# vibhatha/cylon

Hardware: AMD Instinct MI355X
Metric: rows/sec distributed inner-join, 1B×1B int64 keys, at 1/2/4/8 MI355X (higher is better)
Workload: dtype int64 keys / float64 payload; 1 GPU; model=distributed inner join (hash), int64 key + 3 float64 cols, global_batch=1000000000, seq_len=4, parallelism=dp1 (local join), rows_per_relation=1000000000, output_rows=1010151446, key_range=990000000

## Files before the change

cylon_amd/csrc/cylon/kernels/radix_join.hip:

```cpp
#include "radix_common.hpp"

namespace cylon {
namespace hip {

struct PartDigit {
  const int64_t *keys;
  int bits;
  int shift;
  uint32_t mask;
  CYLON_DIGIT_COMMON
  __device__ __forceinline__ uint32_t of_key(int64_t k) const { return (part_of(k, bits) >> shift) & mask; }
  __device__ __forceinline__ uint32_t operator()(int64_t i) const { return of_key(keys[i]); }
  __device__ __forceinline__ uint32_t next_of(uint64_t stored, int nshift, uint32_t nmask, uint64_t) const {
    return (part_of((int64_t)stored, bits) >> nshift) & nmask;
  }
};


struct PartDigitN {
  static constexpr bool kNarrow = true;
  const void *keys;
  int kin4;
  const int64_t *base_src;
  unsigned int *bad;
// ... 168 lines not shown
  const int64_t r0 = t * kRPTile;
#pragma unroll
  for (int u = 0; u < kHTItems; ++u) {
    const int64_t i = r0 + u * kHTThreads + threadIdx.x;
    d[u] = t < ntiles && i < n ? digit(i) : 0xffffffffu;
  }
}
template <class Digit>
__global__ __launch_bounds__(kHTThreads) void k_rp_hist_tiles(Digit digit0, int64_t n, uint32_t nb, int64_t ntiles,
                                                              uint16_t *__restrict__ th) {
  Digit digit = digit0;
  digit.init();
  __shared__ unsigned int hist[kRPMaxBuckets];
  uint32_t d[kHTItems];
  ht_load(digit, n, blockIdx.x, ntiles, d);
  for (int64_t t = blockIdx.x; t < ntiles; t += gridDim.x) {
    for (uint32_t p = threadIdx.x; p < nb; p += blockDim.x) hist[p] = 0;
    __syncthreads();
#pragma unroll
    for (int u = 0; u < kHTItems; ++u)
      if (d[u] != 0xffffffffu) atomicAdd(&hist[d[u]], 1u);
    ht_load(digit, n, t + gridDim.x, ntiles, d);
    __syncthreads();
    for (uint32_t p = threadIdx.x; p < nb; p += blockDim.x) th[t * nb + p] = (uint16_t)hist[p];
    __syncthreads();
  }
}

constexpr int64_t kTsChunk = 512;

__global__ void k_ts_chunk_sums(const uint16_t *__restrict__ th, uint32_t nb, int64_t ntiles,
                                uint32_t *__restrict__ csum) {
  const int64_t c = blockIdx.x, t0 = c * kTsChunk, t1 = t0 + kTsChunk < ntiles ? t0 + kTsChunk : ntiles;
  const uint32_t p = threadIdx.x;
  if (p >= nb) return;
  uint32_t acc = 0;
#pragma unroll 8
  for (int64_t t = t0; t < t1; ++t) acc += th[t * nb + p];
  csum[c * nb + p] = acc;
}

__global__ __launch_bounds__(kRPThreads) void k_ts_chunk_prefix(const uint32_t *__restrict__ csum, uint32_t nb,
                                                                int64_t nchunks, uint32_t *__restrict__ cpre,
                                                                uint32_t *__restrict__ bbase) {
  __shared__ uint32_t wsum[kRPWaves];
  constexpr int B = 16;
  const uint32_t p = threadIdx.x;
  uint32_t acc = 0;
  if (p < nb)
    for (int64_t c0 = 0; c0 < nchunks; c0 += B) {
      uint32_t x[B];
#pragma unroll
      for (int u = 0; u < B; ++u) x[u] = c0 + u < nchunks ? csum[(c0 + u) * nb + p] : 0u;
#pragma unroll
      for (int u = 0; u < B; ++u)
        if (c0 + u < nchunks) {
          cpre[(c0 + u) * nb + p] = acc;
          acc += x[u];
        }
    }
  const uint32_t base = rp_block_exscan<kRPWaves>(p < nb ? acc : 0u, wsum);
  if (p < nb) bbase[p] = base;
}

__global__ void k_ts_offsets(const uint16_t *__restrict__ th, const uint32_t *__restrict__ cpre,
                             const uint32_t *__restrict__ bbase, uint32_t nb, int64_t ntiles,
                             uint32_t *__restrict__ off, const uint32_t *__restrict__ extra) {
  const int64_t c = blockIdx.x, t0 = c * kTsChunk, t1 = t0 + kTsChunk < ntiles ? t0 + kTsChunk : ntiles;
  const uint32_t p = threadIdx.x;
  if (p >= nb) return;
  uint32_t acc = cpre[c * nb + p] + bbase[p] + (extra != nullptr ? extra[p] : 0u);
#pragma unroll 8
  for (int64_t t = t0; t < t1; ++t) {
    off[t * nb + p] = acc;
    acc += th[t * nb + p];
  }
}



template <class Digit, bool W8, int THREADS, int RANK, bool XT = false, bool SLOT = false>
__global__ __launch_bounds__(THREADS) __attribute__((amdgpu_waves_per_eu(4))) void k_rows_pass(
    Digit digit0, int nbits, uint32_t nbuckets, ColSet cols, int64_t n, int64_t rows_per_block, int64_t nblocks,
    const int64_t *__restrict__ bh_scan, TileSched lb) {
  constexpr int WAVES = THREADS / kWave;
  constexpr int TILE = THREADS * kRPItems;
  constexpr int BPT = (kRPMaxBuckets + THREADS - 1) / THREADS;
  Digit digit = digit0;
  digit.init();
  bool narrow_bad = false;
  static_assert(WAVES * kRPMaxBuckets * 2 + TILE * 4 <= TILE * 8, "ranking scratch must fit the stage");
  constexpr bool TICKET = XT || SLOT;
  static_assert(!(XT && SLOT), "one tile schedule");
  static_assert(!SLOT || RANK == kRankBlockAtomic, "slot mode ranks with block atomics (counts in bcnt)");
  const int xhome = TICKET ? xcc_id() : 0;
  __shared__ int64_t running[kRPMaxBuckets];
  __shared__ uint32_t toff[kRPMaxBuckets + 1];
  __shared__ uint64_t ustage[TILE];
  __shared__ uint32_t wsum[WAVES];
  uint16_t *wcnt = reinterpret_cast<uint16_t *>(ustage);
  constexpr bool STABLE = RANK != kRankBlockAtomic;
  uint32_t *bcnt = reinterpret_cast<uint32_t *>(ustage);
  static_assert(WAVES * kRPMaxBuckets * 2 >= kRPMaxBuckets * 4, "block counters must fit the wave counters");
  uint32_t *sdig = reinterpret_cast<uint32_t *>(wcnt + WAVES * kRPMaxBuckets);
  uint8_t *st = reinterpret_cast<uint8_t *>(ustage);
  __shared__ int64_t s_next;
  __shared__ int64_t s_tend[2], s_tr0[2];
  __shared__ int s_tb[2];
  int par = 0;
  bool order_bad = false;
  __shared__ uint32_t tp[SLOT ? kSlotMaxSeg : 1], sss[SLOT ? kSlotMaxSeg : 1], sse[SLOT ? kSlotMaxSeg : 1];
  __shared__ int64_t s_tix, s_thi;
  auto sl_take = [&](int slot) {
    const int64_t t = s_tix;
    if (t >= s_thi) {
      s_tr0[slot] = INT64_MAX / 4;
      s_tend[slot] = 0;
      s_tb[slot] = 0;
      return;
    }
    s_tix = t + ((int64_t)gridDim.x - (blockIdx.x & (kXcds - 1)) + kXcds - 1) / kXcds;
    const int g = sl_segment(tp, lb.sl_nseg, t);
    const int64_t gend = (int64_t)sse[g];
    const int64_t r0 = (int64_t)sss[g] + (t - (int64_t)tp[g]) * TILE;
    s_tr0[slot] = r0;
    s_tend[slot] = r0 + TILE < gend ? r0 + TILE : gend;
    s_tb[slot] = (g >> lb.sl_gshift) * (int)nbuckets * lb.sl_B + (g & lb.sl_gmask);
  };

  const int64_t b = blockIdx.x;
  int64_t begin, end;
  if (SLOT) {
    for (int i = threadIdx.x; i < lb.sl_nseg; i += THREADS) {
      tp[i] = lb.sl_tpre[i];
      sss[i] = lb.sl_ss[i];
      sse[i] = lb.sl_se[i];
    }
    if (threadIdx.x == 0) {
      const int x = blockIdx.x & (kXcds - 1);
      const int g0 = lb.sl_nseg * x / kXcds, g1 = lb.sl_nseg * (x + 1) / kXcds;
      s_tix = (int64_t)lb.sl_tpre[g0] + blockIdx.x / kXcds;
      s_thi = lb.sl_tpre[g1];
    }
    __syncthreads();
    if (threadIdx.x == 0) {
      sl_take(0);
      sl_take(1);
    }
    __syncthreads();
    begin = s_tr0[0];
    end = INT64_MAX / 4;
  } else if (TICKET) {
    if (threadIdx.x == 0) s_next = xt_claim(lb, xhome, TILE, n);
    __syncthreads();
    begin = s_next;
    end = n;
  } else {
    for (uint32_t p = threadIdx.x; p < nbuckets; p += blockDim.x) running[p] = bh_scan[(int64_t)p * nblocks + b];
    begin = b * rows_per_block;
    end = (begin + rows_per_block < n) ? begin + rows_per_block : n;
  }
  const int wave = threadIdx.x / kWave;
  const int lane = lane_id();
  const uint64_t lt = lanemask_lt();
  uint16_t *mycnt = wcnt + wave * nbuckets;
  const int wrow = wave * kWave * kRPItems;

  using KVT = typename std::conditional<Digit::kNarrow, uint32_t, uint64_t>::type;
  KVT kv[kRPItems];
  auto load_key = [&](int64_t i) -> KVT {
    const uint64_t raw = digit.key_at(i);
    if constexpr (Digit::kNarrow) {
      narrow_bad |= digit.too_wide(raw);
      return (KVT)digit.narrow(raw);
    } else {
      return (KVT)raw;
    }
  };
#pragma unroll
  for (int k = 0; k < kRPItems; ++k) {
    const int64_t i = begin + wrow + k * kWave + lane;
    if (i < (SLOT ? s_tend[0] : end)) kv[k] = load_key(i);
  }
  for (int64_t tile = begin, next = 0; tile < end; tile = next) {
    next = tile + TILE;
    const int cnt = SLOT ? (int)(s_tend[par] - tile) : (int)((end - tile) < TILE ? (end - tile) : TILE);
    const uint32_t xoff = XT && threadIdx.x < nbuckets ? lb.xt_off[(tile / TILE) * nbuckets + threadIdx.x] : 0u;
    uint32_t pl[kRPItems];
#pragma unroll
    for (int k = 0; k < kRPItems; ++k) {
      const bool act = wrow + k * kWave + lane < cnt;
      if constexpr (Digit::kNarrow) pl[k] = act ? digit.of_offset(kv[k]) : 0xffffffffu;
      else pl[k] = act ? digit.of_key((int64_t)kv[k]) : 0xffffffffu;
    }
    if (STABLE) {
      for (uint32_t q = threadIdx.x; q < WAVES * nbuckets; q += blockDim.x) wcnt[q] = 0;
    } else {
      for (uint32_t q = threadIdx.x; q < nbuckets; q += blockDim.x) bcnt[q] = 0;
    }
    __syncthreads();
    if (!STABLE) {
#pragma unroll
      for (int k = 0; k < kRPItems; ++k)
        if (pl[k] != 0xffffffffu) pl[k] |= atomicAdd(&bcnt[pl[k]], 1u) << 16;
    } else if (RANK == kRankWaveAtomic) {
      uint32_t *myw = reinterpret_cast<uint32_t *>(mycnt);
#pragma unroll
      for (int k = 0; k < kRPItems; ++k)
        if (pl[k] != 0xffffffffu) {
          const uint32_t p = pl[k], sh = (p & 1u) * 16u;
          pl[k] |= ((atomicAdd(&myw[p >> 1], 1u << sh) >> sh) & 0xffffu) << 16;
        }
    } else
#pragma unroll
    for (int k = 0; k < kRPItems; ++k) {
      const bool active = pl[k] != 0xffffffffu;
      const uint32_t p = active ? pl[k] : 0u;
      uint64_t m = __ballot(active);
      for (int bit = 0; bit < nbits; ++bit) {
        const uint32_t x = (p >> bit) & 1u;
        const uint64_t bb = __ballot(x);
        m &= x ? bb : ~bb;
      }
      const uint32_t rank = (uint32_t)__popcll(m & lt);
      uint32_t base = 0;
      if (active) base = mycnt[p];
      __builtin_amdgcn_wave_barrier();
      if (active && (m & lt) == 0) mycnt[p] = (uint16_t)(base + (uint32_t)__popcll(m));
      __builtin_amdgcn_wave_barrier();
      pl[k] = active ? (((base + rank) << 16) | p) : 0xffffffffu;
    }
    __syncthreads();
    uint32_t sl_c = 0, sl_base = 0;
    if (SLOT && threadIdx.x < nbuckets) {
      sl_c = STABLE ? 0u : bcnt[threadIdx.x];
      if (sl_c) sl_base = atomicAdd(&lb.sl_cursor[(int64_t)s_tb[par] + (int64_t)threadIdx.x * lb.sl_B], sl_c);
    }
    {
      uint32_t loc[BPT];
      uint32_t total = 0;
#pragma unroll
      for (int i = 0; i < BPT; ++i) {
        const uint32_t p = threadIdx.x * BPT + i;
        loc[i] = total;
        uint32_t run = 0;
        if (p < nbuckets) {
          if (STABLE) {
#pragma unroll
            for (int w = 0; w < WAVES; ++w) {
              const uint32_t c = wcnt[w * nbuckets + p];
              wcnt[w * nbuckets + p] = (uint16_t)run;
              run += c;
            }
          } else {
            run = bcnt[p];
          }
        }
        total += run;
      }
      const uint32_t ex = rp_block_exscan<WAVES>(total, wsum);
#pragma unroll
      for (int i = 0; i < BPT; ++i) {
        const uint32_t p = threadIdx.x * BPT + i;
        if (p < nbuckets) toff[p] = ex + loc[i];
      }
      if (threadIdx.x == THREADS - 1) toff[nbuckets] = ex + total;
    }
    __syncthreads();
#pragma unroll
    for (int k = 0; k < kRPItems; ++k) {
      if (pl[k] == 0xffffffffu) continue;
      const uint32_t p = pl[k] & 0xffffu;
      const uint32_t pos = toff[p] + (STABLE ? (uint32_t)wcnt[wave * nbuckets + p] : 0u) + (pl[k] >> 16);
      sdig[pos] = (p << 16) | (uint32_t)(wrow + k * kWave + lane);
      pl[k] = pos;
    }
    if (XT && threadIdx.x < nbuckets) running[threadIdx.x] = xoff;
    if (SLOT && threadIdx.x < nbuckets) {
      const bool fits = (int64_t)sl_base + sl_c <= lb.sl_slot;
      if (sl_c && !fits) atomicOr(lb.sl_overflow, 1u);
      running[threadIdx.x] = fits ? ((int64_t)s_tb[par] + (int64_t)threadIdx.x * lb.sl_B) * lb.sl_slot + sl_base
                                  : lb.sl_nslots * lb.sl_slot;
    }
    __syncthreads();
    constexpr bool PACKDST = false;
    using DstT = typename std::conditional<SLOT, uint32_t, int64_t>::type;
    DstT dst[kRPItems];
#define RP_DEST(q) \
  ((SLOT && PACKDST) ? running[(uint32_t)dst[q] >> 16] + (int64_t)((uint32_t)dst[q] & 0xffffu) : (int64_t)dst[q])
#pragma unroll
    for (int q = 0; q < kRPItems; ++q) {
      const int j = threadIdx.x + q * THREADS;
      if (j < cnt) {
        const uint32_t e = sdig[j], p = e >> 16;
        if constexpr (SLOT && PACKDST) dst[q] = (p << 16) | (uint32_t)(j - (int)toff[p]);
        else dst[q] = (DstT)(running[p] + (j - (int64_t)toff[p]));
        if (cols.check_order && j > 0) {
          const uint32_t f = sdig[j - 1];
          order_bad |= (f >> 16) == p && f > e;
        }
      }
    }
    __syncthreads();
    uint64_t v[kRPItems];
#pragma unroll
    for (int k = 0; k < kRPItems; ++k) v[k] = kv[k];
#pragma unroll 1
    for (int c = 0; c < cols.n; ++c) {
      const int w = cols.width[c];
      uint8_t *out = cols.out[c];
      const uint64_t x = c == 0 ? cols.key_xor : 0ull;
      if (TICKET && c + 1 == cols.n && threadIdx.x == 0) {
        if (!SLOT) s_next = xt_claim(lb, xhome, TILE, n);
      }
      const bool n4 = Digit::kNarrow && c == 0;
      if (n4) {
#pragma unroll
        for (int k = 0; k < kRPItems; ++k)
          if (pl[k] != 0xffffffffu) stw<false>(st, pl[k], 4, v[k] & 0xffffffffull);
      } else {
#pragma unroll
        for (int k = 0; k < kRPItems; ++k)
          if (pl[k] != 0xffffffffu) stw<W8>(st, pl[k], w, v[k] ^ x);
      }
      __syncthreads();
      if (TICKET && c + 1 == cols.n) next = SLOT ? s_tr0[par ^ 1] : s_next;
      if (c + 1 < cols.n) {
        const uint8_t *in = cols.in[c + 1];
        const int w1 = cols.width[c + 1];
        if (in == nullptr) {
#pragma unroll
          for (int k = 0; k < kRPItems; ++k) v[k] = (uint64_t)(tile + wrow + k * kWave + lane);
        } else {
#pragma unroll
          for (int k = 0; k < kRPItems; ++k)
            if (pl[k] != 0xffffffffu) v[k] = ldw<W8>(in, tile + wrow + k * kWave + lane, w1);
        }
      } else {
#pragma unroll
        for (int k = 0; k < kRPItems; ++k) {
          const int64_t i = next + wrow + k * kWave + lane;
          if (i < (SLOT ? s_tend[par ^ 1] : end)) kv[k] = load_key(i);
        }
      }
      if (kNdDigit<Digit> && c == 0 && cols.nd_out != nullptr) {
#pragma unroll
        for (int q = 0; q < kRPItems; ++q) {
          const int j = threadIdx.x + q * THREADS;
          if (j < cnt) {
            const uint64_t kv0 = ldw<W8>(st, j, w);
            const int64_t o = RP_DEST(q);
            stw<W8>(out, o, w, kv0);
            if constexpr (kNdDigit<Digit>)
              cols.nd_out[o] = (uint16_t)digit.next_of(kv0, cols.nd_shift, cols.nd_mask, cols.nd_sub);
          }
        }
      } else if (n4) {
#pragma unroll
        for (int q = 0; q < kRPItems; ++q) {
          const int j = threadIdx.x + q * THREADS;
          if (j < cnt) stw<false>(out, RP_DEST(q), 4, ldw<false>(st, j, 4));
        }
      } else {
#pragma unroll
        for (int q = 0; q < kRPItems; ++q) {
          const int j = threadIdx.x + q * THREADS;
          if (j < cnt) stw<W8>(out, RP_DEST(q), w, ldw<W8>(st, j, w));
        }
      }
      __syncthreads();
    }
#undef RP_DEST
    if (!TICKET)
      for (uint32_t p = threadIdx.x; p < nbuckets; p += blockDim.x) running[p] += toff[p + 1] - toff[p];
    if (SLOT) {
      par ^= 1;
      if (threadIdx.x == 0) sl_take(par ^ 1);
    }
  }
  if (order_bad) atomicOr(cols.order_bad, 1);
  if (Digit::kNarrow && narrow_bad) digit.report_bad();
}

template <class Digit, bool W8, int RANK, bool XT = false, int LBM = 0>
__global__ __launch_bounds__(kRPThreads) __attribute__((amdgpu_waves_per_eu(8))) void k_rows_pass_lean(
    Digit digit, int nbits, uint32_t nbuckets, ColSet cols, int64_t n, int64_t rows_per_block, int64_t nblocks,
    const int64_t *__restrict__ bh_scan, TileSched lb) {
  constexpr int THREADS = kRPThreads, WAVES = THREADS / kWave, TILE = THREADS * kRPItems;
  constexpr bool LBIN = (LBM & 2) != 0, CNT = (LBM & 1) != 0;
  static_assert(LBM == 0 || (XT && (std::is_same<Digit, ImageDigit>::value || std::is_same<Digit, PartDigit>::value)),
                "look-back passes are XT sort / hash-partition passes");
  constexpr int MAXB = LBM ? kLbMaxBuckets : kRPMaxBuckets;
  constexpr int BPT = (MAXB + THREADS - 1) / THREADS;
  static_assert(WAVES * MAXB * 2 + TILE * 4 <= TILE * 8, "ranking scratch must fit the stage");
  __shared__ int64_t running[MAXB];
  __shared__ uint32_t toff[MAXB + 1];
  __shared__ uint64_t ustage[TILE];
  __shared__ uint32_t wsum[WAVES];
  __shared__ uint32_t s_C[LBIN ? kLbChunks + 1 : 1], s_TP[LBIN ? kLbChunks + 2 : 1];
  __shared__ uint32_t lcnt[CNT ? kLbChunks * kLbMaxBuckets / 2 : 1];
  constexpr bool STABLE = RANK != kRankBlockAtomic;
  uint16_t *wcnt = reinterpret_cast<uint16_t *>(ustage);
  uint32_t *bcnt = reinterpret_cast<uint32_t *>(ustage);
  uint32_t *sdig = reinterpret_cast<uint32_t *>(wcnt + WAVES * MAXB);
  uint8_t *st = reinterpret_cast<uint8_t *>(ustage);
  __shared__ int64_t s_next;
  bool order_bad = false;
  (void)nbits;
  constexpr bool TICKET = XT;
  const int xhome = XT ? xcc_id() : 0;
  const uint32_t nbn = cols.nd_mask + 1u;
  const uint32_t lwords = CNT ? kLbChunks * nbn / 2 : 0;
  int since_flush = 0;

  const int64_t b = blockIdx.x;
  int64_t begin, end;
  if (CNT)
    for (uint32_t w = threadIdx.x; w < lwords; w += THREADS) lcnt[w] = 0;
  if (LBIN && threadIdx.x <= kLbChunks) {
    s_C[threadIdx.x] = lb.lb_plan[kLbC + threadIdx.x];
    s_TP[threadIdx.x] = lb.lb_plan[kLbTP + threadIdx.x];
  }
  if (LBIN && threadIdx.x == kLbChunks + 1) s_TP[kLbChunks + 1] = lb.lb_plan[kLbLocal];
  if (TICKET) {
    if (LBIN) __syncthreads();
    if (threadIdx.x == 0) s_next = LBIN ? lb_claim(lb, s_C, s_TP, xhome, TILE, n) : xt_claim(lb, xhome, TILE, n);
    __syncthreads();
    begin = s_next;
    end = n;
  } else {
    for (uint32_t p = threadIdx.x; p < nbuckets; p += THREADS) running[p] = bh_scan[(int64_t)p * nblocks + b];
    begin = b * rows_per_block;
    end = (begin + rows_per_block < n) ? begin + rows_per_block : n;
  }
  const int wave = __builtin_amdgcn_readfirstlane(threadIdx.x / kWave);
  uint16_t *mycnt = wcnt + wave * nbuckets;
  const int wrow = wave * kWave * kRPItems;

  for (int64_t tile = begin, next = 0; tile < end; tile = next) {
    next = tile + TILE;
    int cx = 0;
    if (LBIN)
      while (cx + 1 < kLbChunks && (int64_t)s_C[cx + 1] <= tile) ++cx;
    const int64_t ck = LBIN ? (tile - (int64_t)s_C[cx]) / TILE : 0;
    const int64_t tend = LBIN ? (int64_t)s_C[cx + 1] : end;
    const int cnt = (int)((tend - tile) < TILE ? (tend - tile) : TILE);
    int tx = (int)threadIdx.x;
    asm volatile("" : "+v"(tx));
    const int lane = tx & (kWave - 1);
    const uint32_t xoff = XT && !LBIN && (uint32_t)tx < nbuckets ? lb.xt_off[(tile / TILE) * nbuckets + tx] : 0u;
    uint32_t pl[kRPItems];
    const int64_t *kbase = digit.keys + tile + wrow;
    const int lim = cnt - wrow;
    {
      uint64_t kk[kRPItems];
#pragma unroll
      for (int k = 0; k < kRPItems; ++k) kk[k] = (k * kWave + lane < lim) ? (uint64_t)kbase[k * kWave + lane] : 0ull;
#pragma unroll
      for (int k = 0; k < kRPItems; ++k) pl[k] = (k * kWave + lane < lim) ? digit.of_key((int64_t)kk[k]) : 0xffffffffu;
    }
    if (STABLE) {
      for (uint32_t q = tx; q < WAVES * nbuckets; q += THREADS) wcnt[q] = 0;
    } else {
      for (uint32_t q = tx; q < nbuckets; q += THREADS) bcnt[q] = 0;
    }
    __syncthreads();
    if (!STABLE) {
#pragma unroll
      for (int k = 0; k < kRPItems; ++k)
        if (pl[k] != 0xffffffffu) pl[k] |= atomicAdd(&bcnt[pl[k]], 1u) << 16;
    } else {
      uint32_t *myw = reinterpret_cast<uint32_t *>(mycnt);
#pragma unroll
      for (int k = 0; k < kRPItems; ++k)
        if (pl[k] != 0xffffffffu) {
          const uint32_t p = pl[k], sh = (p & 1u) * 16u;
          pl[k] |= ((atomicAdd(&myw[p >> 1], 1u << sh) >> sh) & 0xffffu) << 16;
        }
    }
    __syncthreads();
    {
      uint32_t loc[BPT];
      uint32_t total = 0;
#pragma unroll
      for (int i = 0; i < BPT; ++i) {
        const uint32_t p = tx * BPT + i;
        loc[i] = total;
        uint32_t run = 0;
        if (p < nbuckets) {
          if (STABLE) {
#pragma unroll
            for (int w = 0; w < WAVES; ++w) {
              const uint32_t c = wcnt[w * nbuckets + p];
              wcnt[w * nbuckets + p] = (uint16_t)run;
              run += c;
            }
          } else {
            run = bcnt[p];
          }
        }
        total += run;
      }
      const uint32_t ex = rp_block_exscan<WAVES>(total, wsum);
#pragma unroll
      for (int i = 0; i < BPT; ++i) {
        const uint32_t p = tx * BPT + i;
        if (p < nbuckets) toff[p] = ex + loc[i];
      }
      if (tx == THREADS - 1) toff[nbuckets] = ex + total;
    }
    __syncthreads();
    const int64_t lgid = LBIN ? (int64_t)s_TP[cx] + ck : 0;
    if (LBIN && (uint32_t)tx < nbuckets) {
      const uint32_t v = (ck == 0 ? 0x80000000u : 0u) | (toff[tx + 1] - toff[tx] + 1u);
      if (s_TP[kLbChunks + 1])
        __hip_atomic_store(&lb.lb_state[lgid * nbuckets + tx], v, __ATOMIC_RELAXED, __HIP_MEMORY_SCOPE_WORKGROUP);
      else
        __hip_atomic_store(&lb.lb_state[lgid * nbuckets + tx], v, __ATOMIC_RELAXED, __HIP_MEMORY_SCOPE_AGENT);
    }
#pragma unroll
    for (int k = 0; k < kRPItems; ++k) {
      if (pl[k] == 0xffffffffu) continue;
      const uint32_t p = pl[k] & 0xffffu;
      const uint32_t pos = toff[p] + (STABLE ? (uint32_t)wcnt[wave * nbuckets + p] : 0u) + (pl[k] >> 16);
      sdig[pos] = (p << 16) | (uint32_t)(wrow + k * kWave + lane);
      pl[k] = pos;
    }
    if (XT && !LBIN && (uint32_t)tx < nbuckets) running[tx] = xoff;
    __syncthreads();
    uint32_t dp[kRPItems];
#pragma unroll
    for (int q = 0; q < kRPItems; ++q) {
      const int j = tx + q * THREADS;
      const uint32_t e = j < cnt ? sdig[j] : 0u, p = e >> 16;
      dp[q] = (p << 16) | (uint32_t)(j - (int)toff[p]);
      if (cols.check_order && j > 0 && j < cnt) {
        const uint32_t f = sdig[j - 1];
        order_bad |= (f >> 16) == p && f > e;
      }
    }
    __syncthreads();
#pragma unroll 1
    for (int c = 0; c < cols.n; ++c) {
      const int w = cols.width[c];
      uint8_t *out = cols.out[c];
      uint64_t v[kRPItems];
      const uint8_t *in = cols.in[c];
      if (in == nullptr) {
        int64_t rbase = tile + wrow;
        asm volatile("" : "+s"(rbase));
#pragma unroll
        for (int k = 0; k < kRPItems; ++k) v[k] = (uint64_t)(rbase + k * kWave + lane);
      } else {
        const uint8_t *ibase = in + (tile + wrow) * (int64_t)w;
#pragma unroll
        for (int k = 0; k < kRPItems; ++k) v[k] = (k * kWave + lane < lim) ? ldw<W8>(ibase, k * kWave + lane, w) : 0ull;
      }
      const uint64_t x = c == 0 ? cols.key_xor : 0ull;
      if (TICKET && !LBIN && c + 1 == cols.n && tx == 0) s_next = xt_claim(lb, xhome, TILE, n);
#pragma unroll
      for (int k = 0; k < kRPItems; ++k)
        if (pl[k] != 0xffffffffu) stw<W8>(st, pl[k], w, v[k] ^ x);
      __syncthreads();
      if (TICKET && !LBIN && c + 1 == cols.n) next = s_next;
      if (LBIN && c == 0 && (uint32_t)tx < nbuckets) {
        const uint32_t own = toff[tx + 1] - toff[tx];
        uint32_t excl = 0;
        if (ck > 0) {
          const int64_t lo = (int64_t)s_TP[cx];
          int64_t j = lgid - 1;
          for (int spin = 0;;) {
            uint32_t w[kLbWindow];
#pragma unroll
            for (int i = 0; i < kLbWindow; ++i)
              w[i] = j - i >= lo ? __hip_atomic_load(&lb.lb_state[(j - i) * nbuckets + tx], __ATOMIC_RELAXED,
                                                     __HIP_MEMORY_SCOPE_AGENT)
                                 : 0u;
            int used = 0;
            bool done = false;
#pragma unroll
            for (int i = 0; i < kLbWindow; ++i) {
              if (done || used < i || w[i] == 0u) continue;
              excl += (w[i] & 0x7fffffffu) - 1u;
              used = i + 1;
              done = (w[i] & 0x80000000u) != 0u;
            }
            if (done) break;
            j -= used;
            if (used == 0) {
              __builtin_amdgcn_s_sleep(1);
              if (++spin > kLbSpinLimit ||
                  ((spin & 255) == 0 && __hip_atomic_load(lb.lb_err, __ATOMIC_RELAXED, __HIP_MEMORY_SCOPE_AGENT))) {
                atomicOr(lb.lb_err, 1u);
                break;
              }
            }
          }
          if (s_TP[kLbChunks + 1])
            __hip_atomic_store(&lb.lb_state[lgid * nbuckets + tx], 0x80000000u | (excl + own + 1u), __ATOMIC_RELAXED,
                               __HIP_MEMORY_SCOPE_WORKGROUP);
          else
            __hip_atomic_store(&lb.lb_state[lgid * nbuckets + tx], 0x80000000u | (excl + own + 1u), __ATOMIC_RELAXED,
                               __HIP_MEMORY_SCOPE_AGENT);
        }
        running[tx] = (int64_t)lb.lb_plan[kLbBase + cx * nbuckets + tx] + excl;
      }
      if (LBIN && c == 0) __syncthreads();
      if (CNT && c == 0) {
        const int xsh = lb.lb_xshift;
#pragma unroll
        for (int q = 0; q < kRPItems; ++q) {
          const int j = tx + q * THREADS;
          if (j < cnt) {
            const uint32_t p = dp[q] >> 16;
            const int64_t o = running[p] + (int64_t)(dp[q] & 0xffffu);
            const uint64_t kv0 = ldw<W8>(st, j, w);
            stw<W8>(out, o, w, kv0);
            uint32_t nd = 0;
            if constexpr (LBM != 0) nd = digit.next_of(kv0, cols.nd_shift, cols.nd_mask, cols.nd_sub);
            const uint32_t cell = (p >> xsh) * nbn + nd;
            atomicAdd(&lcnt[cell >> 1], 1u << ((cell & 1u) << 4));
          }
        }
      } else if (kNdDigit<Digit> && c == 0 && cols.nd_out != nullptr) {
#pragma unroll
        for (int q = 0; q < kRPItems; ++q) {
          const int j = tx + q * THREADS;
          if (j < cnt) {
            const int64_t o = running[dp[q] >> 16] + (int64_t)(dp[q] & 0xffffu);
            const uint64_t kv0 = ldw<W8>(st, j, w);
            stw<W8>(out, o, w, kv0);
            if constexpr (kNdDigit<Digit>)
              cols.nd_out[o] = (uint16_t)digit.next_of(kv0, cols.nd_shift, cols.nd_mask, cols.nd_sub);
          }
        }
      } else {
#pragma unroll
        for (int q = 0; q < kRPItems; ++q) {
          const int j = tx + q * THREADS;
          if (j < cnt) stw<W8>(out, running[dp[q] >> 16] + (int64_t)(dp[q] & 0xffffu), w, ldw<W8>(st, j, w));
        }
      }
      __syncthreads();
    }
    if (!TICKET)
      for (uint32_t p = tx; p < nbuckets; p += THREADS) running[p] += toff[p + 1] - toff[p];
    if (LBIN) {
      if (tx == 0) s_next = lb_claim(lb, s_C, s_TP, xhome, TILE, n);
      __syncthreads();
      next = s_next;
    }
    if (CNT && ++since_flush == 7) {
      lb_flush<THREADS>(lcnt, lb.lb_gcnt + (int64_t)blockIdx.x * (2 * lwords), lwords);
      since_flush = 0;
    }
  }
  if (CNT && since_flush > 0) lb_flush<THREADS>(lcnt, lb.lb_gcnt + (int64_t)blockIdx.x * (2 * lwords), lwords);
  if (order_bad) atomicOr(cols.order_bad, 1);
}

struct RPGeometry {
  int64_t nblocks, rows_per_block;
};

static int rp_threads(int ncols, bool cheap_rank) { return ncols <= 2 && !cheap_rank ? 512 : 1024; }

template <int THREADS, bool PACKED16>
__global__ __launch_bounds__(THREADS) void k_lane_order_check(int rounds, unsigned long long *bad) {
  constexpr int WORDS = PACKED16 ? kRPMaxBuckets / 2 : kRPMaxBuckets;
  __shared__ uint32_t cnt[(THREADS / kWave) * WORDS];
  const int wave = threadIdx.x / kWave, lane = lane_id();
  const uint64_t lt = lanemask_lt();
  uint32_t *mine = cnt + wave * WORDS;
// ... 1047 lines not shown
```

Measured before the change: 23.27 billion rows/s.

## Software-pipeline column loads with scatter drains for full tiles in slot row pass

Adds a fast path for full tiles in the slotted 8-byte row-pass kernel. The next column's global loads (and the next tile's keys on the last column) are issued before the current column is drained from shared memory to its scattered output. The aim is to hide global-load latency behind the scatter stores instead of serialising load, stage and store for each column. The cost is more registers held live and duplicated code paths. The tail tile with the next row clamped to the current row also needs care to stay correct.

```diff
diff --git a/cylon_amd/csrc/cylon/kernels/radix_join.hip b/cylon_amd/csrc/cylon/kernels/radix_join.hip
--- a/cylon_amd/csrc/cylon/kernels/radix_join.hip
+++ b/cylon_amd/csrc/cylon/kernels/radix_join.hip
@@ -494,6 +494,82 @@
       }
     }
     __syncthreads();
+    if (SLOT && W8 && cnt == TILE) {
+      const int64_t row0 = tile + wrow + lane;
+      auto drain = [&](int c, auto n4) {
+        uint8_t *out = cols.out[c];
+        if constexpr (decltype(n4)::value) {
+#pragma unroll
+          for (int q = 0; q < kRPItems; ++q)
+            stw<false>(out, (int64_t)dst[q], 4, ldw<false>(st, threadIdx.x + q * THREADS, 4));
+        } else {
+#pragma unroll
+          for (int q = 0; q < kRPItems; ++q)
+            stw<true>(out, (int64_t)dst[q], 8, ldw<true>(st, threadIdx.x + q * THREADS, 8));
+        }
+      };
+      auto step = [&](int c, auto n4) {
+        const uint64_t *in = reinterpret_cast<const uint64_t *>(cols.in[c + 1]) + row0;
+        uint64_t x[kRPItems];
+#pragma unroll
+        for (int k = 0; k < kRPItems; ++k) x[k] = in[k * kWave];
+        drain(c, n4);
+        __syncthreads();
+#pragma unroll
+        for (int k = 0; k < kRPItems; ++k) stw<true>(st, pl[k], 8, x[k]);
+        __syncthreads();
+      };
+      auto last = [&](auto n4) {
+        next = s_tr0[par ^ 1];
+        const int64_t nrow0 = next + wrow + lane, nend = s_tend[par ^ 1];
+        const int cl = cols.n - 1;
+        if constexpr (Digit::kNarrow) {
+          if (digit.kin4) {
+            const uint32_t *kp = reinterpret_cast<const uint32_t *>(digit.keys);
+#pragma unroll
+            for (int k = 0; k < kRPItems; ++k) kv[k] = kp[(nrow0 + k * kWave < nend ? nrow0 : row0) + k * kWave];
+            drain(cl, n4);
+#pragma unroll
+            for (int k = 0; k < kRPItems; ++k) asm volatile("" : "+v"(kv[k]));
+          } else {
+            const int64_t *kp = reinterpret_cast<const int64_t *>(digit.keys);
+            uint64_t r[kRPItems];
+#pragma unroll
+            for (int k = 0; k < kRPItems; ++k)
+              r[k] = (uint64_t)kp[(nrow0 + k * kWave < nend ? nrow0 : row0) + k * kWave];
+            drain(cl, n4);
+#pragma unroll
+            for (int k = 0; k < kRPItems; ++k) {
+              narrow_bad |= nrow0 + k * kWave < nend && digit.too_wide(r[k]);
+              kv[k] = (KVT)digit.narrow(r[k]);
+            }
+          }
+        } else {
+#pragma unroll
+          for (int k = 0; k < kRPItems; ++k)
+            kv[k] = (KVT)digit.key_at((nrow0 + k * kWave < nend ? nrow0 : row0) + k * kWave);
+          drain(cl, n4);
+        }
+        __syncthreads();
+      };
+      using N4 = std::integral_constant<bool, Digit::kNarrow>;
+      if constexpr (Digit::kNarrow) {
+#pragma unroll
+        for (int k = 0; k < kRPItems; ++k) stw<false>(st, pl[k], 4, (uint64_t)kv[k]);
+      } else {
+#pragma unroll
+        for (int k = 0; k < kRPItems; ++k) stw<true>(st, pl[k], 8, (uint64_t)kv[k] ^ cols.key_xor);
+      }
+      __syncthreads();
+      if (cols.n == 1) {
+        last(N4{});
+      } else {
+        step(0, N4{});
+#pragma unroll 1
+        for (int c = 1; c + 1 < cols.n; ++c) step(c, std::false_type{});
+        last(std::false_type{});
+      }
+    } else {
     uint64_t v[kRPItems];
 #pragma unroll
     for (int k = 0; k < kRPItems; ++k) v[k] = kv[k];
@@ -561,6 +637,7 @@
         }
       }
       __syncthreads();
+    }
     }
 #undef RP_DEST
     if (!TICKET)
```

New measurement: 24.99 billion rows/s, median of 6. +7.4%, better.
